# intel/QAT-ZSTD-Plugin

Hardware: AMD Instinct MI355X
Metric: input MB/s via ZSTD_compress2 L1 128KiB blocks @1/2/4/8 GPU; ratio vs sw zstd (higher is better)
Workload: dtype u8

## Files before the change

include/qzstd_hip.h:

```cpp
#ifndef QZSTD_HIP_H
#define QZSTD_HIP_H

#include <stddef.h>
#include <stdint.h>

#if defined(__cplusplus)
extern "C" {
#endif

#define QZSTD_HIP_BLOCK_MAX (1u << 17)
#define QZSTD_HIP_NSEQ_ERROR 0xFFFFFFFFu
#define QZSTD_HIP_SRC_ALIGN 16u

typedef struct {
    uint32_t tableSize;
    uint32_t tileLog;
    uint32_t capLen;
    uint32_t minMatch;
    uint32_t farLog1;
    uint32_t farLog2;
    uint32_t lazy;
    uint32_t backExt;
    uint32_t nearTab;
    uint32_t window;
// ... 31 lines not shown
size_t qzstd_hip_lds_bytes(int level, uint32_t maxBlockLen);

#ifndef QZ_RING
#define QZ_RING 32768u
#endif
#define QZSTD_HIP_RING_MIRROR 128u
#ifndef QZ_CHAIN_TABLE
#define QZ_CHAIN_TABLE 5888u
#endif
#define QZSTD_HIP_LDS_BASE 16u
#define QZSTD_HIP_LDS_CTRL 64u
#define QZSTD_HIP_LDS_SVC 96u
#define QZSTD_HIP_LDS_MAX 163840u

int qzstd_hip_device_count(void);
int qzstd_hip_device_name(int device, char *buf, size_t bufLen);
void *qzstd_hip_malloc(int device, size_t bytes);
void qzstd_hip_free(int device, void *dptr);
void *qzstd_hip_host_alloc(size_t bytes);
void *qzstd_hip_host_device_ptr(void *hptr);
void qzstd_hip_host_free(void *hptr);
void *qzstd_hip_stream_create(int device);
void qzstd_hip_stream_destroy(int device, void *stream);
int qzstd_hip_stream_sync(int device, void *stream);
int qzstd_hip_stream_query(int device, void *stream);
int qzstd_hip_stream_wait(int device, void *stream, unsigned timeoutMs);
int qzstd_hip_memcpy_h2d(int device, void *stream, void *dst, const void *src, size_t bytes);
int qzstd_hip_copy_in(int device, void *stream, void *dst, const void *src_dev, size_t bytes);
int qzstd_hip_memcpy_d2h(int device, void *stream, void *dst, const void *src, size_t bytes);
int qzstd_hip_memset(int device, void *stream, void *dst, int value, size_t bytes);
int qzstd_hip_memcpy2d_d2h(int device, void *stream, void *dst, size_t dpitch, const void *src, size_t spitch,
                           size_t width, size_t height);

size_t qzstd_hip_workspace_bytes(int level, uint32_t nBlocks, uint32_t maxBlockLen);
int qzstd_hip_find_sequences(int device, void *stream, int level, const void *d_src,
                             const qzstd_hip_block_t *d_blocks, uint32_t nBlocks,
                             uint32_t maxBlockLen, void *d_seqs, uint32_t *d_nseq,
                             void *d_work, size_t workBytes);

int qzstd_hip_occupancy(int device, int level);

#define QZSTD_HIP_NSEQ_REJECTED 0xFFFFFFFEu
#define QZSTD_HIP_NSEQ_STAGING 0xFFFFFFFCu
int qzstd_hip_service_progressive(int device);
#define QZSTD_HIP_SVC_MAX_ITEMS 32u
#define QZSTD_HIP_SVC_MAX_SLOTS 1024u
typedef struct {
    const void *hSrc;
    void *dSrc;
    void *hSeqs;
    uint32_t *hCount;
    uint32_t srcLen, itemBytes, nItems, seqCapPerItem;
    uint32_t slot;
    uint32_t epoch;
    void *dWork;
} qzstd_hip_svc_req_t;
#ifndef QZSTD_HIP_CHAIN_ENTRY_LINKS
#define QZSTD_HIP_CHAIN_ENTRY_LINKS 4u
#endif
#define QZSTD_HIP_SVC_WORK_BYTES ((size_t)QZSTD_HIP_BLOCK_MAX * (8u * QZSTD_HIP_CHAIN_ENTRY_LINKS + 4u) + (size_t)QZSTD_HIP_SVC_MAX_ITEMS * QZ_CHAIN_TABLE * 4u)
int qzstd_hip_service_submit(int device, int level, const qzstd_hip_svc_req_t *req);
int qzstd_hip_service_stop(int device);
int qzstd_hip_service_poke(int device, int level);
void qzstd_hip_service_mark_broken(int device);
int qzstd_hip_service_info(int device, unsigned long out[8]);
int qzstd_hip_service_debug(int device, unsigned long out[8]);
// ... 12 lines not shown
```

qat-zstd-plugin_amd/csrc/qzstd_kernels.hip:

```cpp
#include <hip/hip_runtime.h>

#include <stdint.h>
#include <stdio.h>
#include <stdlib.h>
#include <string.h>

#include <atomic>
#include <mutex>
#include <sched.h>
#include <time.h>
#include <sys/syscall.h>
#include <unistd.h>

#include "qzstd_hip.h"
#include "qzstd_hip_device.h"

#define QZ_PRIO(n) do { if (!CHAIN) __builtin_amdgcn_s_setprio(n); } while (0)

namespace {

constexpr int kMatchWaves = 8;
constexpr int kMatchThreads = kMatchWaves * 64;
constexpr int kThreads = kMatchThreads + 64;
constexpr uint32_t kTileLog = 9;
constexpr uint32_t kTile = 1u << kTileLog;
constexpr uint32_t kWin = kTile >> 6;
constexpr uint32_t kTagBits = 14;
constexpr uint32_t kTagMask = (1u << kTagBits) - 1u;
constexpr uint32_t kPrime1 = 2654435761u;
constexpr uint32_t kPrime2 = 0x85EBCA77u;
constexpr uint32_t kNone = 0xFFFFFFFFu;
constexpr uint32_t kRing = QZ_RING;
constexpr uint32_t kRingMask = kRing - 1u;
constexpr uint32_t kMirror = QZSTD_HIP_RING_MIRROR;
constexpr uint32_t kLook = 4608u;
constexpr uint32_t kNear = kRing - kLook - 3u * kTile - 1024u;
static_assert((kRing & kRingMask) == 0u && kRing >= 16384u, "the ring is a power of two of at least 16 KiB");
constexpr size_t kLdsPerCu = QZSTD_HIP_LDS_MAX;
constexpr uint32_t kEL = QZSTD_HIP_CHAIN_ENTRY_LINKS;
constexpr uint32_t kEQ = QZSTD_HIP_CHAIN_ENTRY_LINKS / 4u;
static_assert(kEL == 4u || kEL == 8u, "chain entries hold four or eight links");
constexpr uint32_t kLdsBase = QZSTD_HIP_LDS_BASE;
constexpr uint32_t kLagT = 2u;

struct LaunchArgs {
    const uint8_t *src;
    const qzstd_hip_block_t *blocks;
    uint4 *seqs;
    uint32_t *nseq;
    qzstd_hip_profile_t prof;
    uint4 *chain;
    uint32_t chainStride;
    uint32_t chainEntries;
    uint32_t pwWords;
    uint32_t orderedLds;
#ifdef QZ_DEBUG_DUMP
    uint32_t dbg;
#endif
};

typedef unsigned long long u64;

#ifdef QZ_DEBUG_DUMP
#define QZ_ABLATED(bit) (args.dbg & (bit))
#define QZ_DBG args.dbg
#else
#define QZ_ABLATED(bit) false
#define QZ_DBG 0u
#endif

#define QZ_BARRIER_LDS() asm volatile("s_waitcnt lgkmcnt(0)\n\ts_barrier" ::: "memory")

#define QZ_RLX_AGENT __ATOMIC_RELAXED, __HIP_MEMORY_SCOPE_AGENT
#define QZ_RLX_SYSTEM __ATOMIC_RELAXED, __HIP_MEMORY_SCOPE_SYSTEM

__device__ __forceinline__ uint32_t rdlane(uint32_t v, uint32_t l) { return (uint32_t)__builtin_amdgcn_readlane((int)v, (int)l); }
__device__ __forceinline__ uint32_t rdfirst(uint32_t v) { return (uint32_t)__builtin_amdgcn_readfirstlane((int)v); }
__device__ __forceinline__ u64 below(uint32_t c) { return c >= 64u ? ~0ull : ((1ull << c) - 1ull); }
__device__ __forceinline__ uint32_t umin(uint32_t a, uint32_t b) { return a < b ? a : b; }
__device__ __forceinline__ uint32_t umax(uint32_t a, uint32_t b) { return a > b ? a : b; }
__device__ __forceinline__ uint32_t umax3(uint32_t a, uint32_t b, uint32_t c) { return umax(umax(a, b), c); }

typedef const __attribute__((address_space(3))) uint32_t *LdsWords;
typedef const __attribute__((address_space(1))) uint32_t *HbmWords;
struct Src {
    LdsWords ring;
    HbmWords g;
// ... 614 lines not shown
                const bool in = vk && slotK == s0;
                const u64 grp = __ballot(in);
                const u64 lower = grp & below(lane);
                if (in && lower) predLane = 63u - (uint32_t)__builtin_clzll(lower);
                rem &= ~grp;
            }
            const uint32_t fromLane = (uint32_t)__shfl((int)mineK, (int)predLane);
            P1[64u * k + lane] = vk ? (predLane != lane ? fromLane : prd) : 0u;
        }
    }
}

struct HistShare {
    uint32_t *flags;
    uint32_t item;
    uint32_t epoch;
    uint32_t spinLimit;
    uint32_t nItems;
    uint32_t *tabFlags;
    uint32_t *linkFlags;
    uint32_t *tabs;
};
constexpr uint32_t kSvcTabStride = QZ_CHAIN_TABLE;
static_assert((uint32_t)kMatchWaves * kPvStride <= QZ_CHAIN_TABLE, "the deferred parse's eight windows of parse words must fit in the head table (QZ_CHAIN_TABLE)");

template <bool HAS_LONG, bool REP, bool CHAIN, bool TURNS, bool NEAR, bool DEFER = false>
__device__ __forceinline__ uint32_t qz_item(const LaunchArgs &args, const qzstd_hip_block_t &blk, const uint8_t *gsrc, uint4 *out,
                                            uint4 *chainB, uint32_t *p1B, const HistShare hsh)
{
    extern __shared__ __attribute__((aligned(16))) uint8_t smem[];
    const uint32_t tid = threadIdx.x;
    const uint32_t lane = tid & 63u;
    const uint32_t wave = rdfirst(tid >> 6);
    const bool matcher = wave < (uint32_t)kMatchWaves;
    const uint32_t n = blk.srcLen;
    const qzstd_hip_profile_t pf = args.prof;
    const uint32_t nh = n >= pf.hashBytes ? n - pf.hashBytes + 1u : 0u;
    const uint32_t nTiles = (nh + kTile - 1u) >> kTileLog;
    const uint32_t itEnd = (DEFER && !CHAIN) ? nTiles : nTiles + kLagT;
    static_assert(kNear + kLagT * kTile + 4u <= kRing - kLook, "the ring no longer holds a near source when its tile is parsed / emitted");
    const uint32_t tabShift = (uint32_t)__builtin_clz(pf.tableSize) + 1u, longShift = pf.longSize ? (uint32_t)__builtin_clz(pf.longSize) + 1u : 31u;
    const uint32_t firstTile = blk.parseFrom >> kTileLog;
    if (blk.parseFrom != 0u && (pf.segLog == 0u || (blk.parseFrom & ((1u << pf.segLog) - 1u)) != 0u || blk.parseFrom >= n)) {
        return QZSTD_HIP_NSEQ_ERROR;
    }
    if (NEAR && n > kRing) return QZSTD_HIP_NSEQ_ERROR;
    if (DEFER && args.pwWords != 0u && ((n + kTile - 1u) & ~(kTile - 1u)) > args.pwWords) return QZSTD_HIP_NSEQ_ERROR;
    if (DEFER && CHAIN && args.chainEntries != 0u && ((n + kTile - 1u) & ~(kTile - 1u)) * kEQ > args.chainEntries) return QZSTD_HIP_NSEQ_ERROR;

    uint8_t *smemI = (uint8_t *)(__attribute__((address_space(3))) uint8_t *)kLdsBase;
    if ((uint32_t)(uintptr_t)(__attribute__((address_space(3))) uint8_t *)smem != 0u) {
        return QZSTD_HIP_NSEQ_ERROR;
    }
    uint32_t *ring32 = reinterpret_cast<uint32_t *>(smemI);
    uint4 *ring128 = reinterpret_cast<uint4 *>(smemI);
    uint32_t *tbl = reinterpret_cast<uint32_t *>(smemI + kRing + kMirror);
    uint32_t *tblL = tbl + pf.tableSize;
    uint32_t *nearTab = tblL + pf.longSize;
    uint32_t *srec = nearTab + kTile;
    uint32_t *pv = srec + kLagT * kWin * kSrecWords;
    uint32_t *turnCtr = pv + kLagT * kPvStride;
    uint32_t *P1odd = turnCtr + QZSTD_HIP_LDS_CTRL / 4u;
    const uint4 *g128 = reinterpret_cast<const uint4 *>(gsrc);
    Src src;
    src.ring = (LdsWords)ring32;
    src.g = (HbmWords)reinterpret_cast<const uint32_t *>(gsrc);
    src.nearLimit = NEAR ? 0xFFFFFFFFu : kNear;
    const uint32_t nPad = (n + 15u) & ~15u;

    const uint32_t itBegin = firstTile;
    const uint32_t histEnd = itBegin << kTileLog;
    const uint32_t hi = umin(nPad, histEnd + kLook + (itBegin ? 0u : kTile));
    const uint32_t lo = hi > kRing ? (hi - kRing + 15u) & ~15u : 0u;
    constexpr uint32_t kStep = (uint32_t)kThreads * 16u;
    const uint32_t hashEnd = CHAIN ? 0u : histEnd;
    uint32_t fo = (hashEnd ? 0u : lo) + tid * 16u;
    uint4 fa0 = make_uint4(0u, 0u, 0u, 0u), fb0 = fa0, fa1 = fa0, fb1 = fa0;
    if (fo < hi) { fa0 = g128[fo >> 4]; if (fo < hashEnd) fb0 = g128[(fo >> 4) + 1u]; }
    if (fo + kStep < hi) { fa1 = g128[(fo + kStep) >> 4]; if (fo + kStep < hashEnd) fb1 = g128[((fo + kStep) >> 4) + 1u]; }
    for (uint32_t i = tid; i < pf.tableSize + pf.longSize; i += kThreads) tbl[i] = 0u;
    if (!(CHAIN && itBegin != 0u)) {
        for (uint32_t i = tid; i < kTile; i += kThreads) nearTab[i] = 0xFFFFFFFFu;
        for (uint32_t i = tid; i < kLagT * kWin * kSrecWords + kLagT * kPvStride + QZSTD_HIP_LDS_CTRL / 4u; i += kThreads) srec[i] = 0u;
    }
    const bool sharedHist = CHAIN && hsh.flags != nullptr && hsh.nItems > 1u && pf.tableSize <= kSvcTabStride;
    if (itBegin != 0u || sharedHist) __syncthreads();
    if (sharedHist) {
        constexpr uint32_t kGroup = 4096u;
        uint32_t *hist = ring32;
        uint32_t *link = ring32 + kGroup;
        const uint32_t a0 = blk.parseFrom, b0 = n, k = hsh.item;
        auto wait_for = [&](uint32_t *fl) -> bool {
            if (wave == 0u) {
                uint32_t spins = 0u, ok = 1u;
                for (;;) {
                    const bool there = lane >= k || __hip_atomic_load(&fl[lane], QZ_RLX_AGENT) == hsh.epoch;
                    if (__all(there)) break;
                    if (++spins > hsh.spinLimit) { ok = 0u; break; }
                    __builtin_amdgcn_s_sleep(2);
                }
                __builtin_amdgcn_fence(__ATOMIC_ACQUIRE, "agent");
                if (lane == 0u) turnCtr[2] = ok;
            }
            __syncthreads();
            const bool ok = rdfirst(turnCtr[2]) != 0u;
            __syncthreads();
            return ok;
        };
        auto hash_group = [&](uint32_t g0) {
            if (tid < 256u) {
                const uint32_t c = g0 + tid * 16u;
                uint4 ha = make_uint4(0u, 0u, 0u, 0u), hb = ha;
                if (c < b0) { ha = g128[c >> 4]; hb = g128[(c >> 4) + 1u]; }
                const uint32_t W[5] = { ha.x, ha.y, ha.z, ha.w, hb.x };
                const uint32_t segEc = seg_end(pf, c, n);
                uint32_t st16[16];
// ... 13 lines not shown
            hash_group(g0);
            QZ_BARRIER_LDS();
            if (wave == 2u || wave == 3u) {
                const uint32_t nW = (umin(kGroup, b0 - g0) + 63u) >> 6;
                const uint32_t par = wave & 1u;
                for (uint32_t w0 = 0; w0 < nW; w0 += 16u) {
                    uint32_t st[16], pred[16];
#pragma unroll
                    for (uint32_t j = 0; j < 16u; j++) st[j] = w0 + j < nW ? hist[64u * (w0 + j) + lane] : kNone;
#pragma unroll
                    for (uint32_t j = 0; j < 16u; j++) {
                        const uint32_t pos = g0 + 64u * (w0 + j) + lane;
                        const bool mine = st[j] != kNone && (st[j] & 1u) == par;
                        pred[j] = 0u;
                        if (mine) pred[j] = args.orderedLds != 0u ? atomicMax(&tbl[st[j] & 0xFFFFu], ((pos + 1u) << kTagBits) | (st[j] >> 16))
                                                                   : chain_insert_window(tbl, st[j], ((pos + 1u) << kTagBits) | (st[j] >> 16), lane, false);
                        else if (args.orderedLds == 0u) (void)chain_insert_window(tbl, kNone, 0u, lane, false);
                    }
#pragma unroll
                    for (uint32_t j = 0; j < 16u; j++)
                        if (w0 + j < nW && (st[j] == kNone || (st[j] & 1u) == par)) link[64u * (w0 + j) + lane] = pred[j];
                }
            }
            QZ_BARRIER_LDS();
            if (tid < 512u) {
#pragma unroll
                for (uint32_t j = 0; j < 2u; j++)
                    if (g0 + (j * 512u + tid) * 4u < b0) reinterpret_cast<uint4 *>(p1B + g0)[j * 512u + tid] = reinterpret_cast<const uint4 *>(link)[j * 512u + tid];
            }
            QZ_BARRIER_LDS();
        }
        {
            uint32_t *mine = hsh.tabs + (size_t)k * kSvcTabStride;
            for (uint32_t i = tid; i < pf.tableSize; i += kThreads) __hip_atomic_store(&mine[i], tbl[i], QZ_RLX_AGENT);
            asm volatile("s_waitcnt vmcnt(0)" ::: "memory");
            __syncthreads();
            if (tid == 0u) __hip_atomic_store(&hsh.tabFlags[k], hsh.epoch, QZ_RLX_AGENT);
        }
        if (!wait_for(hsh.tabFlags)) return QZSTD_HIP_NSEQ_ERROR;
        for (uint32_t i = tid; i < pf.tableSize; i += kThreads) {
            uint32_t m = 0u;
            for (uint32_t j = 0; j < k; j++) m = umax(m, hsh.tabs[(size_t)j * kSvcTabStride + i]);
            tbl[i] = m;
        }
        __syncthreads();
        for (uint32_t g0 = a0; g0 < b0; g0 += kGroup) {
            hash_group(g0);
            QZ_BARRIER_LDS();
            if (tid < 512u) {
#pragma unroll
                for (uint32_t j = 0; j < 8u; j++) {
                    const uint32_t i = j * 512u + tid, pos = g0 + i;
                    if (pos < b0) {
                        uint32_t l1 = p1B[pos];
                        const uint32_t st = hist[i];
                        if (l1 == 0u && st != kNone) l1 = tbl[st & 0xFFFFu];
                        __hip_atomic_store(&p1B[pos], l1, QZ_RLX_AGENT);
                    }
                }
            }
            QZ_BARRIER_LDS();
        }
        asm volatile("s_waitcnt vmcnt(0)" ::: "memory");
        __syncthreads();
        if (tid == 0u) __hip_atomic_store(&hsh.linkFlags[k], hsh.epoch, QZ_RLX_AGENT);
        if (!wait_for(hsh.linkFlags)) return QZSTD_HIP_NSEQ_ERROR;
        constexpr uint32_t kCh = 16u / kEL;
        for (uint32_t p0 = a0 + tid; p0 < b0; p0 += kCh * (uint32_t)kThreads) {
            uint32_t e[kEL][kCh];
#pragma unroll
            for (uint32_t i = 0; i < kCh; i++) { const uint32_t pp = p0 + i * (uint32_t)kThreads; e[0][i] = pp < b0 ? __hip_atomic_load(&p1B[pp], QZ_RLX_AGENT) : 0u; }
#pragma unroll
            for (uint32_t d = 1; d < kEL; d++)
#pragma unroll
                for (uint32_t i = 0; i < kCh; i++) e[d][i] = e[d - 1u][i] ? __hip_atomic_load(&p1B[(e[d - 1u][i] >> kTagBits) - 1u], QZ_RLX_AGENT) : 0u;
#pragma unroll
            for (uint32_t i = 0; i < kCh; i++) {
                const uint32_t pp = p0 + i * (uint32_t)kThreads;
                if (pp < b0) {
                    u64 *w = reinterpret_cast<u64 *>(chainB + (size_t)pp * kEQ);
#pragma unroll
                    for (uint32_t d = 0; d < kEL; d += 2u) __hip_atomic_store(w + d / 2u, (u64)e[d][i] | ((u64)e[d + 1u][i] << 32), QZ_RLX_AGENT);
                }
            }
        }
        asm volatile("s_waitcnt vmcnt(0)" ::: "memory");
        __syncthreads();
        if (tid == 0u) __hip_atomic_store(&hsh.flags[k], hsh.epoch, QZ_RLX_AGENT);
        if (!wait_for(hsh.flags)) return QZSTD_HIP_NSEQ_ERROR;
        for (uint32_t i = tid; i < kTile; i += kThreads) nearTab[i] = 0xFFFFFFFFu;
        for (uint32_t i = tid; i < kLagT * kWin * kSrecWords + kLagT * kPvStride + QZSTD_HIP_LDS_CTRL / 4u; i += kThreads) srec[i] = 0u;
    } else if (CHAIN && itBegin != 0u) {
        constexpr uint32_t kGroup = 4096u;
        static_assert(kGroup * 8u <= kRing, "two words per position of a group in the ring's LDS");
        uint32_t *hist = ring32;
        uint32_t *link = ring32 + kGroup;
        const uint32_t nGroups = (histEnd + kGroup - 1u) / kGroup;
        uint4 ha = make_uint4(0u, 0u, 0u, 0u), hb = ha;
        if (tid < 256u && tid * 16u < histEnd) { ha = g128[tid]; hb = g128[tid + 1u]; }
        for (uint32_t g = 0; g < nGroups && !QZ_ABLATED(2048u); g++) {
            const uint32_t g0 = g * kGroup;
            if (tid < 256u) {
                const uint32_t c = g0 + tid * 16u;
                const uint32_t W[5] = { ha.x, ha.y, ha.z, ha.w, hb.x };
                const uint32_t segEc = seg_end(pf, c, n);
                uint32_t st16[16];
#pragma unroll
                for (uint32_t k = 0; k < 16u; k++) {
                    const uint32_t v = (k & 3u) ? __builtin_amdgcn_alignbyte(W[(k >> 2) + 1u], W[k >> 2], k & 3u) : W[k >> 2];
                    const uint32_t mixH = v * kPrime1;
                    const bool ok = c + k < histEnd && c + k + 4u <= segEc;
                    st16[k] = ok ? (__umulhi(mixH, pf.tableSize) | (((mixH >> 3) & kTagMask) << 16)) : kNone;
                }
#pragma unroll
                for (uint32_t k = 0; k < 4u; k++)
                    reinterpret_cast<uint4 *>(hist)[tid * 4u + k] = make_uint4(st16[4u * k], st16[4u * k + 1u], st16[4u * k + 2u], st16[4u * k + 3u]);
                const uint32_t cn = c + kGroup;
                ha = hb = make_uint4(0u, 0u, 0u, 0u);
                if (cn < histEnd) { ha = g128[cn >> 4]; hb = g128[(cn >> 4) + 1u]; }
            }
            QZ_BARRIER_LDS();
            if (wave == 2u || wave == 3u) {
                const uint32_t nW = umin(kGroup, histEnd - g0) >> 6;
                const uint32_t par = wave & 1u;
// ... 2 lines not shown
                        uint32_t st[16], pred[16];
#pragma unroll
                        for (uint32_t k = 0; k < 16u; k++) st[k] = hist[64u * (w0 + k) + lane];
#pragma unroll
                        for (uint32_t k = 0; k < 16u; k++) {
                            const uint32_t pos = g0 + 64u * (w0 + k) + lane;
                            pred[k] = 0u;
                            if (st[k] != kNone && (st[k] & 1u) == par) pred[k] = atomicMax(&tbl[st[k] & 0xFFFFu], ((pos + 1u) << kTagBits) | (st[k] >> 16));
                        }
#pragma unroll
                        for (uint32_t k = 0; k < 16u; k++)
                            if (st[k] == kNone || (st[k] & 1u) == par) link[64u * (w0 + k) + lane] = pred[k];
                    }
                } else {
                    for (uint32_t w = 0; w < nW; w++) {
                        const uint32_t st = hist[64u * w + lane];
                        const uint32_t pos = g0 + 64u * w + lane;
                        const bool mine = st != kNone && (st & 1u) == par;
                        const uint32_t pred = chain_insert_window(tbl, mine ? st : kNone, ((pos + 1u) << kTagBits) | (st >> 16), lane, false);
                        if (mine || st == kNone) link[64u * w + lane] = pred;
                    }
                }
            }
            QZ_BARRIER_LDS();
            if (tid < 512u && !QZ_ABLATED(1024u)) {
#pragma unroll
                for (uint32_t k = 0; k < 2u; k++)
                    if (g0 + (k * 512u + tid) * 4u < histEnd) reinterpret_cast<uint4 *>(p1B + g0)[k * 512u + tid] = reinterpret_cast<const uint4 *>(link)[k * 512u + tid];
            }
            QZ_BARRIER_LDS();
        }
        constexpr uint32_t kChase = 32u / kEL;
        const uint32_t chaseFrom = hsh.flags ? histEnd - histEnd / hsh.item : 0u;
        for (uint32_t p0 = chaseFrom + tid; p0 < histEnd && !QZ_ABLATED(512u); p0 += kChase * (uint32_t)kThreads) {
            uint32_t e[kEL][kChase];
#pragma unroll
            for (uint32_t i = 0; i < kChase; i++) { const uint32_t pp = p0 + i * (uint32_t)kThreads; e[0][i] = pp < histEnd ? p1B[pp] : 0u; }
#pragma unroll
            for (uint32_t d = 1; d < kEL; d++)
#pragma unroll
                for (uint32_t i = 0; i < kChase; i++) e[d][i] = e[d - 1u][i] ? p1B[(e[d - 1u][i] >> kTagBits) - 1u] : 0u;
#pragma unroll
            for (uint32_t i = 0; i < kChase; i++) {
                const uint32_t pp = p0 + i * (uint32_t)kThreads;
                if (pp < histEnd) {
                    if (hsh.flags) {
                        u64 *w = reinterpret_cast<u64 *>(chainB + (size_t)pp * kEQ);
#pragma unroll
                        for (uint32_t d = 0; d < kEL; d += 2u) __hip_atomic_store(w + d / 2u, (u64)e[d][i] | ((u64)e[d + 1u][i] << 32), QZ_RLX_AGENT);
                    } else {
#pragma unroll
                        for (uint32_t j = 0; j < kEL / 4u; j++) chainB[(size_t)pp * kEQ + j] = make_uint4(e[4u * j][i], e[4u * j + 1u][i], e[4u * j + 2u][i], e[4u * j + 3u][i]);
                    }
                }
            }
        }
        if (hsh.flags) {
            asm volatile("s_waitcnt vmcnt(0)" ::: "memory");
            __syncthreads();
            if (wave == 0u) {
                if (lane == 0u) __hip_atomic_store(&hsh.flags[hsh.item], hsh.epoch, QZ_RLX_AGENT);
                uint32_t spins = 0u, ok = 1u;
                for (;;) {
                    const bool there = lane == 0u || lane >= hsh.item || __hip_atomic_load(&hsh.flags[lane], QZ_RLX_AGENT) == hsh.epoch;
                    if (__all(there)) break;
                    if (++spins > hsh.spinLimit) { ok = 0u; break; }
                    __builtin_amdgcn_s_sleep(2);
                }
                __builtin_amdgcn_fence(__ATOMIC_ACQUIRE, "agent");
                if (lane == 0u) turnCtr[2] = ok;
            }
            __syncthreads();
            if (rdfirst(turnCtr[2]) == 0u) return QZSTD_HIP_NSEQ_ERROR;
        }
        __syncthreads();
        for (uint32_t i = tid; i < kTile; i += kThreads) nearTab[i] = 0xFFFFFFFFu;
        for (uint32_t i = tid; i < kLagT * kWin * kSrecWords + kLagT * kPvStride + QZSTD_HIP_LDS_CTRL / 4u; i += kThreads) srec[i] = 0u;
    }
    {
        const uint32_t hiMaskH = pf.hashBytes >= 8 ? 0xFFFFFFFFu : ((1u << (8u * (pf.hashBytes - 4u))) - 1u);
        for (; fo < hi; fo += kStep) {
            uint4 fa2 = make_uint4(0u, 0u, 0u, 0u), fb2 = fa2;
            const uint32_t o2 = fo + 2u * kStep;
            if (o2 < hi) { fa2 = g128[o2 >> 4]; if (o2 < hashEnd) fb2 = g128[(o2 >> 4) + 1u]; }
            if (fo >= lo) {
                const uint32_t r = ring_dw(fo) << 2;
                ring128[r >> 4] = fa0;
                if (r < kMirror) ring128[(kRing + r) >> 4] = fa0;
            }
            if (fo < hashEnd) {
                const uint32_t W[6] = { fa0.x, fa0.y, fa0.z, fa0.w, fb0.x, fb0.y };
                const uint32_t segEc = seg_end(pf, fo, n);
#pragma unroll
                for (uint32_t k = 0; k < 16u; k++) {
                    const uint32_t p = fo + k;
                    if (p + pf.hashBytes <= segEc) {
                        const uint32_t v = __builtin_amdgcn_alignbyte(W[(k >> 2) + 1u], W[k >> 2], k & 3u);
                        const uint32_t w = __builtin_amdgcn_alignbyte(W[(k >> 2) + 2u], W[(k >> 2) + 1u], k & 3u);
                        const uint32_t mixH = (v * kPrime1) ^ __umul24(pf.hashBytes > 4 ? w & hiMaskH : 0u, kPrime2 & 0xFFFFFFu);
                        atomicMax(&tbl[mixH >> tabShift], ((p + 1u) << kTagBits) | ((mixH >> 3) & kTagMask));
                        if (HAS_LONG && p + 8u <= segEc) {
                            const uint32_t m8 = (v * kPrime1) ^ (w * kPrime2);
                            atomicMax(&tblL[m8 >> longShift], ((p + 1u) << kTagBits) | ((m8 >> 3) & kTagMask));
                        }
                    }
                }
            }
            fa0 = fa1; fb0 = fb1; fa1 = fa2; fb1 = fb2;
        }
        if (itBegin != 0u && TURNS && !CHAIN && tid == 0u) *turnCtr = itBegin * (uint32_t)kMatchWaves;
        if (itBegin == 0u)
            for (uint32_t o = hi + tid * 16u; o < kTile + kLook; o += kThreads * 16u) {
                ring128[o >> 4] = make_uint4(0u, 0u, 0u, 0u);
                if (o < kMirror) ring128[(kRing + o) >> 4] = make_uint4(0u, 0u, 0u, 0u);
            }
    }
    __syncthreads();

    if (DEFER && !matcher) __builtin_amdgcn_endpgm();
    if (!matcher) {
        if (!QZ_ABLATED(32u)) __builtin_amdgcn_s_setprio(3);
#ifndef QZ_PARSE_SPLIT
#define QZ_PARSE_SPLIT 3
#endif
        constexpr uint32_t kSplit = QZ_PARSE_SPLIT;
#ifdef QZ_DEBUG_DUMP
        u64 pI1 = 0, pW1 = 0, pI2 = 0, pW2 = 0, tQ = __builtin_amdgcn_s_memtime();
#define QZ_PLAP(acc) { const u64 tN = __builtin_amdgcn_s_memtime(); acc += tN - tQ; tQ = tN; }
#else
#define QZ_PLAP(acc)
#endif
        uint32_t nseqEnd, anchorEnd;
        if (REP) {
            RepState st = { blk.parseFrom, blk.parseFrom, 0u, 0u, 0u, 0u, pf.segLog ? blk.parseFrom >> pf.segLog : 0u };
            for (uint32_t it = itBegin; it < itEnd; it++) {
                const bool work = it >= 1u && it - 1u < nTiles && it - 1u >= firstTile && !QZ_ABLATED(1u);
                const uint32_t k = it - 1u, base = k << kTileLog;
                uint32_t *pvT = pv + (k % kLagT) * kPvStride, *srecT = srec + (k % kLagT) * kWin * kSrecWords;
                if (work) {
                    st.tileSeq = st.nseq;
                    if (lane == 0u) srecT[0] = st.nseq;
                    if (!CHAIN) parse_rep_span<false>(pf, src, pvT, base, base + 64u * kSplit, n, nh, lane, st);
                }
                if (CHAIN && it == itBegin && it < nTiles) chain_insert_tile(pf, src, tbl, (it & 1u) ? P1odd : nearTab, it << kTileLog, n, nh, lane, args.orderedLds != 0u);
                QZ_PLAP(pI1)
// ... 573 lines not shown
                        const uint32_t maxb = umin(umin(umin(pf.backExt, lit), q), pm & (kSeg - 1u));
                        uint32_t b = 0;
                        if (maxb) {
                            const uint32_t pb = rd32u(src, pm - 4u, false);
                            uint32_t qb;
                            if (q < qs + 4u) qb = q >= 4u ? rd32u(src, q - 4u, true) : rd32u(src, 0u, true) << (8u * (4u - q));
                            else qb = rd32u(src, q - 4u, false);
                            const uint32_t x = pb ^ qb;
                            b = umin(x ? (uint32_t)__builtin_clz(x) >> 3 : 4u, maxb);
                        }
                        const uint32_t idx = total + before + k;
                        if (idx < blk.seqCap) store_entry(out, idx, off, lit - b, len + b, blk.mark);
                    }
                }
                total += all;
                anchorCarry = anchorOut;
            }
            __syncthreads();
        }
        if (wave != 0u) return 0u;
        uint32_t count = total + 1u;
        if (lane == 0 && total < blk.seqCap) store_entry(out, total, 0u, n - anchorCarry, 0u, blk.mark);
        if (count + 1u >= blk.seqCap) count = QZSTD_HIP_NSEQ_ERROR;
        return count;
    }
    return 0u;
}

#ifndef QZ_WAVES_PER_EU
#define QZ_WAVES_PER_EU 5
#endif
#define QZ_OCCUPANCY __attribute__((amdgpu_waves_per_eu(QZ_WAVES_PER_EU)))
template <bool HAS_LONG, bool REP, bool CHAIN, bool TURNS, bool NEAR>
__global__ __launch_bounds__(kThreads) QZ_OCCUPANCY void qzstd_find_sequences_kernel(LaunchArgs args)
{
    const qzstd_hip_block_t blk = args.blocks[blockIdx.x];
    const uint32_t count = qz_item<HAS_LONG, REP, CHAIN, TURNS, NEAR, true>(args, blk, args.src + blk.srcOff, args.seqs + blk.seqOff,
                                                              CHAIN ? args.chain + (size_t)blockIdx.x * args.chainStride : nullptr,
                                                              reinterpret_cast<uint32_t *>(args.chain + (size_t)blockIdx.x * args.chainStride + args.chainEntries),
                                                              HistShare{ nullptr, 0u, 0u, 0u, 0u, nullptr, nullptr, nullptr });
    asm volatile("s_waitcnt vmcnt(0)" ::: "memory");
    __syncthreads();
    if (threadIdx.x == 0u)
        __hip_atomic_store(args.nseq + blockIdx.x, count, __ATOMIC_RELEASE, __HIP_MEMORY_SCOPE_SYSTEM);
}

constexpr uint32_t kSvcQueue = 4096u;
constexpr uint32_t kSvcRing = 256u;
constexpr uint32_t kSvcMaxItems = 32u;
constexpr uint32_t kSvcSlots = 1024u;
constexpr uint32_t kSvcRejected = 0xFFFFFFFEu;

struct SvcDev {
    u64 items[kSvcQueue][8];
    uint32_t head;
    uint32_t done;
    uint32_t quit;
    uint32_t spinFails;
    uint32_t started;
    uint32_t taken;
    uint32_t pad[2];
    uint32_t sliceFlag[kSvcSlots][kSvcMaxItems];
    uint32_t histFlag[kSvcSlots][kSvcMaxItems];
    uint32_t tabFlag[kSvcSlots][kSvcMaxItems];
    uint32_t linkFlag[kSvcSlots][kSvcMaxItems];
};

struct SvcHost {
    u64 ring[kSvcRing][8];
    uint32_t state;
    uint32_t quitReq;
    u64 consumed;
    u64 itemsDone;
    uint32_t spinFails;
    uint32_t pad;
    u64 dbg[8];
};
// ... 678 lines not shown
    {
        static std::mutex attrMu;
        static bool attrDone[64];
        std::lock_guard<std::mutex> g(attrMu);
        if (phys(device) < 0) return fail_msg("qzstd_hip_find_sequences: device index out of range");
        if (!attrDone[device]) {
            size_t most = 0;
            for (int l = 1; l <= 12; l++) {
                const size_t b = qzstd_hip_lds_bytes(l, QZSTD_HIP_BLOCK_MAX);
                if (b > most) most = b;
            }
            for (int v = 0; v < 24; v++) {
                const void *f = variants[v / 12][(v / 6) % 2][(v / 3) % 2][v % 3];
                if (f) QZ_CHECK(hipFuncSetAttribute(f, hipFuncAttributeMaxDynamicSharedMemorySize, (int)most),
                                "hipFuncSetAttribute(MaxDynamicSharedMemorySize)");
            }
            attrDone[device] = true;
        }
    }
    a.chain = nullptr;
    a.pwWords = 0;
    a.chainStride = 0;
    a.chainEntries = 0;
    a.orderedLds = 0;
    if (a.prof.chainDepth) {
        a.orderedLds = (uint32_t)probe_lds_order(device, phys(device));
        const size_t need = qzstd_hip_workspace_bytes(level, nBlocks, maxBlockLen);
        if (!d_work || workBytes < need) return fail_msg("qzstd_hip_find_sequences: workspace missing or too small (qzstd_hip_workspace_bytes)");
        a.chain = static_cast<uint4 *>(d_work);
        a.chainStride = (uint32_t)(need / nBlocks / sizeof(uint4));
        a.chainEntries = (uint32_t)(need / nBlocks / (4u * QZSTD_HIP_CHAIN_ENTRY_LINKS + 4u)) * kEQ;
    } else {
        const size_t need = qzstd_hip_workspace_bytes(level, nBlocks, maxBlockLen);
        if (!d_work || workBytes < need || need == 0) return fail_msg("qzstd_hip_find_sequences: workspace missing or too small (qzstd_hip_workspace_bytes)");
        a.chain = static_cast<uint4 *>(d_work);
        a.chainStride = (uint32_t)(need / nBlocks / sizeof(uint4));
        a.pwWords = (uint32_t)(need / nBlocks / 33u * 8u);
    }
    if (a.prof.segLog != 12u) return fail_msg("qzstd_hip_find_sequences: unsupported profile (the deferred parse of a launch works on 4 KiB segments)");
    a.src = static_cast<const uint8_t *>(d_src);
    a.blocks = d_blocks;
    a.seqs = static_cast<uint4 *>(d_seqs);
    a.nseq = d_nseq;
#ifdef QZ_DEBUG_DUMP
    { const char *ab = getenv("QZSTD_HIP_ABLATE"); a.dbg = ab ? (uint32_t)atoi(ab) : 0u; }
#endif
#ifdef QZ_DEBUG_DUMP
    size_t ldsLaunch = lds;
    { const char *pad = getenv("QZSTD_HIP_LDS_PAD"); if (pad) ldsLaunch += (size_t)atoi(pad); }
#else
    const size_t ldsLaunch = lds;
#endif
    const dim3 grid(nBlocks), wg(kThreads);
    const int nearK = maxBlockLen <= kRing ? 1 : 0;
    const void *kernel = variants[nearK][a.prof.longSize ? 1 : 0][a.prof.repWin ? 1 : 0][a.prof.chainDepth ? 2 : (a.prof.subTileLog ? 1 : 0)];
    void *kargs[1] = { &a };
    if (!kernel) return fail_msg("qzstd_hip_find_sequences: unsupported profile (no kernel variant)");
    if (!a.prof.chainDepth && ((a.prof.tableSize & (a.prof.tableSize - 1u)) != 0u || (a.prof.longSize & (a.prof.longSize - 1u)) != 0u || a.prof.hashBytes > 7u))
        return fail_msg("qzstd_hip_find_sequences: unsupported profile (tables below the chain levels are powers of two, hashBytes <= 7)");
    QZ_CHECK(hipLaunchKernel(kernel, grid, wg, kargs, ldsLaunch, (hipStream_t)stream), "launch qzstd_find_sequences_kernel");
    QZ_CHECK(hipGetLastError(), "launch qzstd_find_sequences_kernel");
    if (big && bigLock.owns_lock()) {
        Service &sv = g_svc[device];
        int k = sv.bigNext;
        for (int tries = 0; tries < Service::kBig && sv.bigUsed[k]; tries++) {
            if (hipEventQuery(sv.bigEv[k]) != hipErrorNotReady) { (void)hipGetLastError(); sv.bigUsed[k] = false; break; }
            k = (k + 1) % Service::kBig;
        }
        if (sv.bigUsed[k]) { (void)hipEventSynchronize(sv.bigEv[k]); (void)hipGetLastError(); }
        sv.bigNext = (k + 1) % Service::kBig;
        if (!sv.bigEv[k] && hipEventCreateWithFlags(&sv.bigEv[k], hipEventDisableTiming) != hipSuccess) { sv.bigEv[k] = nullptr; (void)hipGetLastError(); }
        if (sv.bigEv[k] && hipEventRecord(sv.bigEv[k], (hipStream_t)stream) == hipSuccess) { sv.bigUsed[k] = true; sv.bigLds[k] = lds; }
        else (void)hipGetLastError();
    }
    return 0;
}

int qzstd_hip_occupancy(int device, int level)
{
    qzstd_hip_profile_t p;
    if (qzstd_hip_profile_for_level(level, QZSTD_HIP_BLOCK_MAX, &p)) return fail_msg("qzstd_hip_occupancy: bad level");
    const size_t lds = qzstd_hip_lds_bytes(level, QZSTD_HIP_BLOCK_MAX);
    QZ_SET_DEVICE(device);
    const void *k;
    if (p.chainDepth) k = p.repWin ? reinterpret_cast<const void *>(qzstd_find_sequences_kernel<false, true, true, true, false>) : reinterpret_cast<const void *>(qzstd_find_sequences_kernel<false, false, true, true, false>);
    else if (p.longSize) k = p.repWin ? reinterpret_cast<const void *>(qzstd_find_sequences_kernel<true, true, false, false, false>) : reinterpret_cast<const void *>(qzstd_find_sequences_kernel<true, false, false, false, false>);
    else if (p.subTileLog) k = p.repWin ? reinterpret_cast<const void *>(qzstd_find_sequences_kernel<false, true, false, true, false>) : reinterpret_cast<const void *>(qzstd_find_sequences_kernel<false, false, false, true, false>);
    else k = p.repWin ? reinterpret_cast<const void *>(qzstd_find_sequences_kernel<false, true, false, false, false>) : reinterpret_cast<const void *>(qzstd_find_sequences_kernel<false, false, false, false, false>);
    (void)hipFuncSetAttribute(k, hipFuncAttributeMaxDynamicSharedMemorySize, (int)lds);
    int n = 0;
    QZ_CHECK(hipOccupancyMaxActiveBlocksPerMultiprocessor(&n, k, kThreads, lds), "hipOccupancyMaxActiveBlocksPerMultiprocessor");
    return n;
}

}

namespace {

const void *svc_worker_variant(const qzstd_hip_profile_t &p)
{
#define QZ_W(L, R, C, T) reinterpret_cast<const void *>(qzstd_service_worker<L, R, C, T, false>)
    if (p.chainDepth) return p.repWin ? QZ_W(false, true, true, true) : QZ_W(false, false, true, true);
    if (p.longSize) return p.repWin ? QZ_W(true, true, false, false) : QZ_W(true, false, false, false);
    if (p.repWin) return p.subTileLog ? QZ_W(false, true, false, true) : QZ_W(false, true, false, false);
    return p.subTileLog ? QZ_W(false, false, false, true) : QZ_W(false, false, false, false);
#undef QZ_W
}

int svc_level_index(int level)
{
    const int l = level & ~QZSTD_HIP_LEVEL_REPCODES;
    return (l >= 1 && l <= 12) ? (l - 1) + ((level & QZSTD_HIP_LEVEL_REPCODES) ? 12 : 0) : -1;
}

int svc_launch_locked(int device, Service &s, int level)
{
    const SvcConfig &cfg = svc_config();
    LaunchArgs a;
    memset(&a, 0, sizeof(a));
    if (qzstd_hip_profile_for_level(level, QZSTD_HIP_BLOCK_MAX, &a.prof)) return fail_msg("service: bad level");
    static const bool multiOn = [] { const char *v = getenv("QZSTD_HIP_SERVICE_MULTI"); return !(v && atoi(v) == 0); }();
    const bool multi = multiOn && a.prof.longSize == 0u;
    const void *worker = multi ? reinterpret_cast<const void *>(qzstd_service_worker<false, false, false, false, true>) : svc_worker_variant(a.prof);
    size_t lds = qzstd_hip_lds_bytes(level, QZSTD_HIP_BLOCK_MAX);
// ... 561 lines not shown
```

qat-zstd-plugin_amd/csrc/qzstd_profile.c:

```c
#include "qzstd_hip.h"

#include <string.h>


int qzstd_hip_profile_for_level(int level, size_t blockSize, qzstd_hip_profile_t *out)
{
    const int repcodes = (level & QZSTD_HIP_LEVEL_REPCODES) != 0;
    level &= ~QZSTD_HIP_LEVEL_REPCODES;
    if (level < 1 || level > 12 || !out) return -1;
    memset(out, 0, sizeof(*out));
    (void)blockSize;
    {
        const int chains = level >= 5;
        out->tableSize = chains ? QZ_CHAIN_TABLE : (level >= 3 ? 16384u : 8192u);
        out->longSize = (!chains && level >= 3) ? 8192u : 0u;
        out->tileLog = 9;
#ifndef QZ_CAP_HI
#define QZ_CAP_HI 48u
#endif
#ifndef QZ_CAP_MID
#define QZ_CAP_MID 48u
#endif
#ifndef QZ_DEPTH_HI
#define QZ_DEPTH_HI 40u
#endif
        out->capLen = level >= 9 ? QZ_CAP_HI : (level >= 5 ? QZ_CAP_MID : 48u);
        out->minMatch = 4;
        out->farLog1 = 12;
        out->farLog2 = 16;
        out->lazy = chains ? 4u : 3u;
        out->backExt = 4;
        out->nearTab = chains ? 0u : 1u;
        out->window = 0;
        out->hashBytes = chains ? 4u : 5u;
        out->extLog = 11;
        out->repWin = (repcodes || level >= 10) ? 16u : 0u;
#ifndef QZ_DEPTH_6
#define QZ_DEPTH_6 12u
#endif
        out->chainDepth = level >= 10 ? QZ_DEPTH_HI : (level >= 9 ? 64u : (level >= 7 ? 32u : (level >= 6 ? QZ_DEPTH_6 : (level >= 5 ? 8u : 0u))));
        out->subTileLog = (chains || level == 2) ? 6u : 0u;
        out->segLog = 12u;
    }
    return 0;
}

size_t qzstd_hip_sequence_bound(size_t srcSize)
{
    return srcSize / 3 + 1 + srcSize / 1024 + 1;
}

size_t qzstd_hip_workspace_bytes(int level, uint32_t nBlocks, uint32_t maxBlockLen)
{
    qzstd_hip_profile_t p;
    if (maxBlockLen > QZSTD_HIP_BLOCK_MAX || qzstd_hip_profile_for_level(level, maxBlockLen, &p)) return 0;
    if (!p.chainDepth)
        return (size_t)nBlocks * ((((size_t)maxBlockLen + 511u) & ~(size_t)511u) / 8u * 33u);
    return (size_t)nBlocks * (((size_t)maxBlockLen + 511u) & ~(size_t)511u) * (4u * QZSTD_HIP_CHAIN_ENTRY_LINKS + 4u);
}

size_t qzstd_hip_lds_bytes(int level, uint32_t maxBlockLen)
{
    qzstd_hip_profile_t p;
    size_t need;
    const size_t lag = 2u;
    if (maxBlockLen > QZSTD_HIP_BLOCK_MAX || qzstd_hip_profile_for_level(level, maxBlockLen, &p)) return 0;
    need = (size_t)QZ_RING + QZSTD_HIP_RING_MIRROR
           + 4u * p.tableSize
           + 4u * p.longSize
           + (4u << p.tileLog)
           + lag * ((4u << p.tileLog) + 32u)
           + lag * ((1u << p.tileLog) >> 6) * 32u
           + (p.chainDepth ? (4u << p.tileLog) : 0u)
           + QZSTD_HIP_LDS_BASE + QZSTD_HIP_LDS_CTRL + QZSTD_HIP_LDS_SVC;
    return need <= QZSTD_HIP_LDS_MAX ? need : 0;
}
```

Measured before the change: 22540.

## Run non-chain levels as a persistent grid of matcher-only workgroups

For levels without hash chains, the find-sequences kernel now launches at most as many workgroups as fit resident on the device, capped at 512. Each workgroup loops over blocks with a grid stride and reuses one workspace region, which shrinks the workspace to at most 512 regions. The workgroup size drops to the eight matcher waves, removing the extra service wave, and the loop strides inside the item code use the new thread count. This aims to cut launch and scheduling overhead and raise occupancy. In exchange, each region is now reused serially, and load balance across the fixed grid may be uneven.

Result: slower. 21310 (-5.5%).

```diff
diff --git a/include/qzstd_hip.h b/include/qzstd_hip.h
--- a/include/qzstd_hip.h
+++ b/include/qzstd_hip.h
@@ -87,6 +87,7 @@
 int qzstd_hip_memcpy2d_d2h(int device, void *stream, void *dst, size_t dpitch, const void *src, size_t spitch,
                            size_t width, size_t height);
 
+#define QZSTD_HIP_RESIDENT_MAX 512u
 size_t qzstd_hip_workspace_bytes(int level, uint32_t nBlocks, uint32_t maxBlockLen);
 int qzstd_hip_find_sequences(int device, void *stream, int level, const void *d_src,
                              const qzstd_hip_block_t *d_blocks, uint32_t nBlocks,
diff --git a/qat-zstd-plugin_amd/csrc/qzstd_kernels.hip b/qat-zstd-plugin_amd/csrc/qzstd_kernels.hip
--- a/qat-zstd-plugin_amd/csrc/qzstd_kernels.hip
+++ b/qat-zstd-plugin_amd/csrc/qzstd_kernels.hip
@@ -53,6 +53,7 @@
     uint32_t chainStride;
     uint32_t chainEntries;
     uint32_t pwWords;
+    uint32_t nBlocks;
     uint32_t orderedLds;
 #ifdef QZ_DEBUG_DUMP
     uint32_t dbg;
@@ -733,7 +734,8 @@
     const uint32_t tid = threadIdx.x;
     const uint32_t lane = tid & 63u;
     const uint32_t wave = rdfirst(tid >> 6);
-    const bool matcher = wave < (uint32_t)kMatchWaves;
+    constexpr uint32_t kT = (DEFER && !CHAIN) ? (uint32_t)kMatchThreads : (uint32_t)kThreads;
+    const bool matcher = kT == (uint32_t)kMatchThreads || wave < (uint32_t)kMatchWaves;
     const uint32_t n = blk.srcLen;
     const qzstd_hip_profile_t pf = args.prof;
     const uint32_t nh = n >= pf.hashBytes ? n - pf.hashBytes + 1u : 0u;
@@ -773,16 +775,16 @@
     const uint32_t histEnd = itBegin << kTileLog;
     const uint32_t hi = umin(nPad, histEnd + kLook + (itBegin ? 0u : kTile));
     const uint32_t lo = hi > kRing ? (hi - kRing + 15u) & ~15u : 0u;
-    constexpr uint32_t kStep = (uint32_t)kThreads * 16u;
+    constexpr uint32_t kStep = kT * 16u;
     const uint32_t hashEnd = CHAIN ? 0u : histEnd;
     uint32_t fo = (hashEnd ? 0u : lo) + tid * 16u;
     uint4 fa0 = make_uint4(0u, 0u, 0u, 0u), fb0 = fa0, fa1 = fa0, fb1 = fa0;
     if (fo < hi) { fa0 = g128[fo >> 4]; if (fo < hashEnd) fb0 = g128[(fo >> 4) + 1u]; }
     if (fo + kStep < hi) { fa1 = g128[(fo + kStep) >> 4]; if (fo + kStep < hashEnd) fb1 = g128[((fo + kStep) >> 4) + 1u]; }
-    for (uint32_t i = tid; i < pf.tableSize + pf.longSize; i += kThreads) tbl[i] = 0u;
+    for (uint32_t i = tid; i < pf.tableSize + pf.longSize; i += kT) tbl[i] = 0u;
     if (!(CHAIN && itBegin != 0u)) {
-        for (uint32_t i = tid; i < kTile; i += kThreads) nearTab[i] = 0xFFFFFFFFu;
-        for (uint32_t i = tid; i < kLagT * kWin * kSrecWords + kLagT * kPvStride + QZSTD_HIP_LDS_CTRL / 4u; i += kThreads) srec[i] = 0u;
+        for (uint32_t i = tid; i < kTile; i += kT) nearTab[i] = 0xFFFFFFFFu;
+        for (uint32_t i = tid; i < kLagT * kWin * kSrecWords + kLagT * kPvStride + QZSTD_HIP_LDS_CTRL / 4u; i += kT) srec[i] = 0u;
     }
     const bool sharedHist = CHAIN && hsh.flags != nullptr && hsh.nItems > 1u && pf.tableSize <= kSvcTabStride;
     if (itBegin != 0u || sharedHist) __syncthreads();
@@ -862,13 +864,13 @@
         }
         {
             uint32_t *mine = hsh.tabs + (size_t)k * kSvcTabStride;
-            for (uint32_t i = tid; i < pf.tableSize; i += kThreads) __hip_atomic_store(&mine[i], tbl[i], QZ_RLX_AGENT);
+            for (uint32_t i = tid; i < pf.tableSize; i += kT) __hip_atomic_store(&mine[i], tbl[i], QZ_RLX_AGENT);
             asm volatile("s_waitcnt vmcnt(0)" ::: "memory");
             __syncthreads();
             if (tid == 0u) __hip_atomic_store(&hsh.tabFlags[k], hsh.epoch, QZ_RLX_AGENT);
         }
         if (!wait_for(hsh.tabFlags)) return QZSTD_HIP_NSEQ_ERROR;
-        for (uint32_t i = tid; i < pf.tableSize; i += kThreads) {
+        for (uint32_t i = tid; i < pf.tableSize; i += kT) {
             uint32_t m = 0u;
             for (uint32_t j = 0; j < k; j++) m = umax(m, hsh.tabs[(size_t)j * kSvcTabStride + i]);
             tbl[i] = m;
@@ -896,17 +898,17 @@
         if (tid == 0u) __hip_atomic_store(&hsh.linkFlags[k], hsh.epoch, QZ_RLX_AGENT);
         if (!wait_for(hsh.linkFlags)) return QZSTD_HIP_NSEQ_ERROR;
         constexpr uint32_t kCh = 16u / kEL;
-        for (uint32_t p0 = a0 + tid; p0 < b0; p0 += kCh * (uint32_t)kThreads) {
+        for (uint32_t p0 = a0 + tid; p0 < b0; p0 += kCh * kT) {
             uint32_t e[kEL][kCh];
 #pragma unroll
-            for (uint32_t i = 0; i < kCh; i++) { const uint32_t pp = p0 + i * (uint32_t)kThreads; e[0][i] = pp < b0 ? __hip_atomic_load(&p1B[pp], QZ_RLX_AGENT) : 0u; }
+            for (uint32_t i = 0; i < kCh; i++) { const uint32_t pp = p0 + i * kT; e[0][i] = pp < b0 ? __hip_atomic_load(&p1B[pp], QZ_RLX_AGENT) : 0u; }
 #pragma unroll
             for (uint32_t d = 1; d < kEL; d++)
 #pragma unroll
                 for (uint32_t i = 0; i < kCh; i++) e[d][i] = e[d - 1u][i] ? __hip_atomic_load(&p1B[(e[d - 1u][i] >> kTagBits) - 1u], QZ_RLX_AGENT) : 0u;
 #pragma unroll
             for (uint32_t i = 0; i < kCh; i++) {
-                const uint32_t pp = p0 + i * (uint32_t)kThreads;
+                const uint32_t pp = p0 + i * kT;
                 if (pp < b0) {
                     u64 *w = reinterpret_cast<u64 *>(chainB + (size_t)pp * kEQ);
 #pragma unroll
@@ -918,8 +920,8 @@
         __syncthreads();
         if (tid == 0u) __hip_atomic_store(&hsh.flags[k], hsh.epoch, QZ_RLX_AGENT);
         if (!wait_for(hsh.flags)) return QZSTD_HIP_NSEQ_ERROR;
-        for (uint32_t i = tid; i < kTile; i += kThreads) nearTab[i] = 0xFFFFFFFFu;
-        for (uint32_t i = tid; i < kLagT * kWin * kSrecWords + kLagT * kPvStride + QZSTD_HIP_LDS_CTRL / 4u; i += kThreads) srec[i] = 0u;
+        for (uint32_t i = tid; i < kTile; i += kT) nearTab[i] = 0xFFFFFFFFu;
+        for (uint32_t i = tid; i < kLagT * kWin * kSrecWords + kLagT * kPvStride + QZSTD_HIP_LDS_CTRL / 4u; i += kT) srec[i] = 0u;
     } else if (CHAIN && itBegin != 0u) {
         constexpr uint32_t kGroup = 4096u;
         static_assert(kGroup * 8u <= kRing, "two words per position of a group in the ring's LDS");
@@ -988,17 +990,17 @@
         }
         constexpr uint32_t kChase = 32u / kEL;
         const uint32_t chaseFrom = hsh.flags ? histEnd - histEnd / hsh.item : 0u;
-        for (uint32_t p0 = chaseFrom + tid; p0 < histEnd && !QZ_ABLATED(512u); p0 += kChase * (uint32_t)kThreads) {
+        for (uint32_t p0 = chaseFrom + tid; p0 < histEnd && !QZ_ABLATED(512u); p0 += kChase * kT) {
             uint32_t e[kEL][kChase];
 #pragma unroll
-            for (uint32_t i = 0; i < kChase; i++) { const uint32_t pp = p0 + i * (uint32_t)kThreads; e[0][i] = pp < histEnd ? p1B[pp] : 0u; }
+            for (uint32_t i = 0; i < kChase; i++) { const uint32_t pp = p0 + i * kT; e[0][i] = pp < histEnd ? p1B[pp] : 0u; }
 #pragma unroll
             for (uint32_t d = 1; d < kEL; d++)
 #pragma unroll
                 for (uint32_t i = 0; i < kChase; i++) e[d][i] = e[d - 1u][i] ? p1B[(e[d - 1u][i] >> kTagBits) - 1u] : 0u;
 #pragma unroll
             for (uint32_t i = 0; i < kChase; i++) {
-                const uint32_t pp = p0 + i * (uint32_t)kThreads;
+                const uint32_t pp = p0 + i * kT;
                 if (pp < histEnd) {
                     if (hsh.flags) {
                         u64 *w = reinterpret_cast<u64 *>(chainB + (size_t)pp * kEQ);
@@ -1030,8 +1032,8 @@
             if (rdfirst(turnCtr[2]) == 0u) return QZSTD_HIP_NSEQ_ERROR;
         }
         __syncthreads();
-        for (uint32_t i = tid; i < kTile; i += kThreads) nearTab[i] = 0xFFFFFFFFu;
-        for (uint32_t i = tid; i < kLagT * kWin * kSrecWords + kLagT * kPvStride + QZSTD_HIP_LDS_CTRL / 4u; i += kThreads) srec[i] = 0u;
+        for (uint32_t i = tid; i < kTile; i += kT) nearTab[i] = 0xFFFFFFFFu;
+        for (uint32_t i = tid; i < kLagT * kWin * kSrecWords + kLagT * kPvStride + QZSTD_HIP_LDS_CTRL / 4u; i += kT) srec[i] = 0u;
     }
     {
         const uint32_t hiMaskH = pf.hashBytes >= 8 ? 0xFFFFFFFFu : ((1u << (8u * (pf.hashBytes - 4u))) - 1u);
@@ -1066,7 +1068,7 @@
         }
         if (itBegin != 0u && TURNS && !CHAIN && tid == 0u) *turnCtr = itBegin * (uint32_t)kMatchWaves;
         if (itBegin == 0u)
-            for (uint32_t o = hi + tid * 16u; o < kTile + kLook; o += kThreads * 16u) {
+            for (uint32_t o = hi + tid * 16u; o < kTile + kLook; o += kT * 16u) {
                 ring128[o >> 4] = make_uint4(0u, 0u, 0u, 0u);
                 if (o < kMirror) ring128[(kRing + o) >> 4] = make_uint4(0u, 0u, 0u, 0u);
             }
@@ -1706,17 +1708,21 @@
 #endif
 #define QZ_OCCUPANCY __attribute__((amdgpu_waves_per_eu(QZ_WAVES_PER_EU)))
 template <bool HAS_LONG, bool REP, bool CHAIN, bool TURNS, bool NEAR>
-__global__ __launch_bounds__(kThreads) QZ_OCCUPANCY void qzstd_find_sequences_kernel(LaunchArgs args)
-{
-    const qzstd_hip_block_t blk = args.blocks[blockIdx.x];
-    const uint32_t count = qz_item<HAS_LONG, REP, CHAIN, TURNS, NEAR, true>(args, blk, args.src + blk.srcOff, args.seqs + blk.seqOff,
-                                                              CHAIN ? args.chain + (size_t)blockIdx.x * args.chainStride : nullptr,
-                                                              reinterpret_cast<uint32_t *>(args.chain + (size_t)blockIdx.x * args.chainStride + args.chainEntries),
-                                                              HistShare{ nullptr, 0u, 0u, 0u, 0u, nullptr, nullptr, nullptr });
-    asm volatile("s_waitcnt vmcnt(0)" ::: "memory");
-    __syncthreads();
-    if (threadIdx.x == 0u)
-        __hip_atomic_store(args.nseq + blockIdx.x, count, __ATOMIC_RELEASE, __HIP_MEMORY_SCOPE_SYSTEM);
+__global__ __launch_bounds__(CHAIN ? kThreads : kMatchThreads) QZ_OCCUPANCY void qzstd_find_sequences_kernel(LaunchArgs args)
+{
+    uint4 *const region = args.chain + (size_t)blockIdx.x * args.chainStride;
+    uint32_t b = blockIdx.x;
+    do {
+        const qzstd_hip_block_t blk = args.blocks[b];
+        const uint32_t count = qz_item<HAS_LONG, REP, CHAIN, TURNS, NEAR, true>(args, blk, args.src + blk.srcOff, args.seqs + blk.seqOff,
+                                                                  CHAIN ? region : nullptr, reinterpret_cast<uint32_t *>(region + args.chainEntries),
+                                                                  HistShare{ nullptr, 0u, 0u, 0u, 0u, nullptr, nullptr, nullptr });
+        asm volatile("s_waitcnt vmcnt(0)" ::: "memory");
+        __syncthreads();
+        if (threadIdx.x == 0u)
+            __hip_atomic_store(args.nseq + b, count, __ATOMIC_RELEASE, __HIP_MEMORY_SCOPE_SYSTEM);
+        b += gridDim.x;
+    } while (!CHAIN && b < args.nBlocks);
 }
 
 constexpr uint32_t kSvcQueue = 4096u;
@@ -2461,11 +2467,13 @@
         a.chainEntries = (uint32_t)(need / nBlocks / (4u * QZSTD_HIP_CHAIN_ENTRY_LINKS + 4u)) * kEQ;
     } else {
         const size_t need = qzstd_hip_workspace_bytes(level, nBlocks, maxBlockLen);
+        const uint32_t regions = nBlocks < QZSTD_HIP_RESIDENT_MAX ? nBlocks : QZSTD_HIP_RESIDENT_MAX;
         if (!d_work || workBytes < need || need == 0) return fail_msg("qzstd_hip_find_sequences: workspace missing or too small (qzstd_hip_workspace_bytes)");
         a.chain = static_cast<uint4 *>(d_work);
-        a.chainStride = (uint32_t)(need / nBlocks / sizeof(uint4));
-        a.pwWords = (uint32_t)(need / nBlocks / 33u * 8u);
-    }
+        a.chainStride = (uint32_t)(need / regions / sizeof(uint4));
+        a.pwWords = (uint32_t)(need / regions / 33u * 8u);
+    }
+    a.nBlocks = nBlocks;
     if (a.prof.segLog != 12u) return fail_msg("qzstd_hip_find_sequences: unsupported profile (the deferred parse of a launch works on 4 KiB segments)");
     a.src = static_cast<const uint8_t *>(d_src);
     a.blocks = d_blocks;
@@ -2480,11 +2488,42 @@
 #else
     const size_t ldsLaunch = lds;
 #endif
-    const dim3 grid(nBlocks), wg(kThreads);
     const int nearK = maxBlockLen <= kRing ? 1 : 0;
-    const void *kernel = variants[nearK][a.prof.longSize ? 1 : 0][a.prof.repWin ? 1 : 0][a.prof.chainDepth ? 2 : (a.prof.subTileLog ? 1 : 0)];
+    const int vLong = a.prof.longSize ? 1 : 0, vRep = a.prof.repWin ? 1 : 0, vKind = a.prof.chainDepth ? 2 : (a.prof.subTileLog ? 1 : 0);
+    const void *kernel = variants[nearK][vLong][vRep][vKind];
     void *kargs[1] = { &a };
     if (!kernel) return fail_msg("qzstd_hip_find_sequences: unsupported profile (no kernel variant)");
+    uint32_t groups = nBlocks;
+    if (!a.prof.chainDepth) {
+        static std::mutex resMu;
+        static uint32_t resGroups[64][2][2][2][2];
+        static size_t resLds[64][2][2][2][2];
+        uint32_t r;
+        {
+            std::lock_guard<std::mutex> g(resMu);
+            uint32_t &known = resGroups[device][nearK][vLong][vRep][vKind];
+            size_t &knownLds = resLds[device][nearK][vLong][vRep][vKind];
+            if (known == 0u || knownLds != ldsLaunch) {
+                int perCu = 0, cus = 0;
+                QZ_CHECK(hipOccupancyMaxActiveBlocksPerMultiprocessor(&perCu, kernel, kMatchThreads, ldsLaunch), "hipOccupancyMaxActiveBlocksPerMultiprocessor");
+                QZ_CHECK(hipDeviceGetAttribute(&cus, hipDeviceAttributeMultiprocessorCount, phys(device)), "hipDeviceGetAttribute(MultiprocessorCount)");
+                if (perCu < 1 || cus < 1) return fail_msg("qzstd_hip_find_sequences: the runtime reports no resident workgroup for this kernel");
+                const unsigned long long fit = (unsigned long long)perCu * (unsigned long long)cus;
+                known = fit < QZSTD_HIP_RESIDENT_MAX ? (uint32_t)fit : QZSTD_HIP_RESIDENT_MAX;
+                knownLds = ldsLaunch;
+            }
+            r = known;
+        }
+        static const uint32_t resEnv = [] {
+            const char *v = getenv("QZSTD_HIP_RESIDENT");
+            const long k = v && *v ? atol(v) : 0l;
+            if (k > 0) fprintf(stderr, "qzstd_hip: QZSTD_HIP_RESIDENT=%ld: launches below the chain levels start at most %ld workgroups\n", k, k);
+            return k > 0 ? (uint32_t)(k < (long)QZSTD_HIP_RESIDENT_MAX ? k : (long)QZSTD_HIP_RESIDENT_MAX) : 0u;
+        }();
+        if (resEnv != 0u && resEnv < r) r = resEnv;
+        groups = nBlocks < r ? nBlocks : r;
+    }
+    const dim3 grid(groups), wg(a.prof.chainDepth ? kThreads : kMatchThreads);
     if (!a.prof.chainDepth && ((a.prof.tableSize & (a.prof.tableSize - 1u)) != 0u || (a.prof.longSize & (a.prof.longSize - 1u)) != 0u || a.prof.hashBytes > 7u))
         return fail_msg("qzstd_hip_find_sequences: unsupported profile (tables below the chain levels are powers of two, hashBytes <= 7)");
     QZ_CHECK(hipLaunchKernel(kernel, grid, wg, kargs, ldsLaunch, (hipStream_t)stream), "launch qzstd_find_sequences_kernel");
@@ -2518,7 +2557,7 @@
     else k = p.repWin ? reinterpret_cast<const void *>(qzstd_find_sequences_kernel<false, true, false, false, false>) : reinterpret_cast<const void *>(qzstd_find_sequences_kernel<false, false, false, false, false>);
     (void)hipFuncSetAttribute(k, hipFuncAttributeMaxDynamicSharedMemorySize, (int)lds);
     int n = 0;
-    QZ_CHECK(hipOccupancyMaxActiveBlocksPerMultiprocessor(&n, k, kThreads, lds), "hipOccupancyMaxActiveBlocksPerMultiprocessor");
+    QZ_CHECK(hipOccupancyMaxActiveBlocksPerMultiprocessor(&n, k, p.chainDepth ? kThreads : kMatchThreads, lds), "hipOccupancyMaxActiveBlocksPerMultiprocessor");
     return n;
 }
 
diff --git a/qat-zstd-plugin_amd/csrc/qzstd_profile.c b/qat-zstd-plugin_amd/csrc/qzstd_profile.c
--- a/qat-zstd-plugin_amd/csrc/qzstd_profile.c
+++ b/qat-zstd-plugin_amd/csrc/qzstd_profile.c
@@ -55,7 +55,7 @@
     qzstd_hip_profile_t p;
     if (maxBlockLen > QZSTD_HIP_BLOCK_MAX || qzstd_hip_profile_for_level(level, maxBlockLen, &p)) return 0;
     if (!p.chainDepth)
-        return (size_t)nBlocks * ((((size_t)maxBlockLen + 511u) & ~(size_t)511u) / 8u * 33u);
+        return (size_t)(nBlocks < QZSTD_HIP_RESIDENT_MAX ? nBlocks : QZSTD_HIP_RESIDENT_MAX) * ((((size_t)maxBlockLen + 511u) & ~(size_t)511u) / 8u * 33u);
     return (size_t)nBlocks * (((size_t)maxBlockLen + 511u) & ~(size_t)511u) * (4u * QZSTD_HIP_CHAIN_ENTRY_LINKS + 4u);
 }
 
```
